# discord/lilliput

Measured on NVIDIA H100. Metric: images_per_sec_1080p_jpeg_to_256x256_jpeg_q85, higher is better.
Workload: dtype u8

## Files before the change

### lilliput_b200/csrc/jpeg_huff_parallel.cu

```cuda
#include <cstdlib>

#include "common.cuh"
#include "kernels.cuh"

namespace lp {

__device__ unsigned long long g_huff_phase[8];
#define LP_PHASE_MARK(k)                                             \
    do {                                                             \
        if (threadIdx.x == 0) {                                      \
            const long long now_ = clock64();                        \
            atomicAdd(&g_huff_phase[k], (unsigned long long)(now_ - s_tphase)); \
            s_tphase = now_;                                         \
        }                                                            \
    } while (0)

constexpr uint32_t kMinSubBits = 1024;
constexpr uint32_t kSubPerThread = 1;
#ifndef LP_HUFF_THREADS
#define LP_HUFF_THREADS 512
#endif
constexpr int kHuffThreads = LP_HUFF_THREADS;

__constant__ uint8_t c_zigzag_p[64] = {0,  1,  8,  16, 9,  2,  3,  10, 17, 24, 32, 25, 18, 11, 4,  5,
                                       12, 19, 26, 33, 40, 48, 41, 34, 27, 20, 13, 6,  7,  14, 21, 28,
                                       35, 42, 49, 56, 57, 50, 43, 36, 29, 22, 15, 23, 30, 37, 44, 51,
                                       58, 59, 52, 45, 38, 31, 39, 46, 53, 60, 61, 54, 47, 55, 62, 63};


template <int THREADS>
__device__ __forceinline__ uint32_t block_excl_scan(uint32_t v, uint32_t* total, uint32_t* warp_sums) {
    const int lane = threadIdx.x & 31, wid = threadIdx.x >> 5;
    uint32_t inc = v;
#pragma unroll
    for (int o = 1; o < 32; o <<= 1) {
        const uint32_t t = __shfl_up_sync(0xffffffffu, inc, o);
        if (lane >= o) inc += t;
    }
    if (lane == 31) warp_sums[wid] = inc;
    __syncthreads();
    if (wid == 0) {
        uint32_t s = lane < THREADS / 32 ? warp_sums[lane] : 0;
#pragma unroll
        for (int o = 1; o < 32; o <<= 1) {
            const uint32_t t = __shfl_up_sync(0xffffffffu, s, o);
            if (lane >= o) s += t;
        }
        if (lane < THREADS / 32) warp_sums[lane] = s;
    }
    __syncthreads();
    const uint32_t base = wid ? warp_sums[wid - 1] : 0;
    *total = warp_sums[THREADS / 32 - 1];
    __syncthreads();
    return base + inc - v;
}


__global__ void __launch_bounds__(kHuffThreads)
    jpeg_unstuff_kernel(JpegDecodeItem* items, const uint8_t* scan, uint8_t* clean) {
    __shared__ uint32_t warp_sums[kHuffThreads / 32];
    __shared__ uint32_t s_end;
    __shared__ __align__(16) uint8_t stage[kHuffThreads * 16 + 16];
    JpegDecodeItem& it = items[blockIdx.x];
    const uint8_t* src = scan + it.scan_off;
    const uint32_t len = it.scan_len;
    uint8_t* dst = clean + it.clean_off;
    const int tid = threadIdx.x, lane = tid & 31;
    if (it.restart_interval != 0 || it.nscans != 0) return;
    if (it.status != 0) {
        if (tid == 0) it.clean_len = 0;
        return;
    }
    if (tid == 0) s_end = len;
    __syncthreads();
    const uint32_t mis = (uint32_t)(reinterpret_cast<uintptr_t>(src) & 15);
    const uint8_t* abase = src - mis;
    uint32_t carry = 0;
    uint32_t end = len;
    constexpr uint32_t kTile = kHuffThreads * 16;
    for (uint32_t t0 = 0; t0 < mis + end; t0 += kTile) {
        const uint32_t aoff = t0 + (uint32_t)tid * 16;
        const int64_t i0 = (int64_t)aoff - (int64_t)mis;
        uint4 w = make_uint4(0, 0, 0, 0);
        if (aoff < mis + len + 16) w = *reinterpret_cast<const uint4*>(abase + aoff);
        uint32_t prev = __shfl_up_sync(0xffffffffu, w.w >> 24, 1);
        uint32_t next = __shfl_down_sync(0xffffffffu, w.x & 0xffu, 1);
        if (lane == 0) prev = i0 > 0 ? src[i0 - 1] : 0;
        if (lane == 31) next = (i0 + 16 < (int64_t)len) ? src[i0 + 16] : 0xD9u;
        const uint32_t ws[4] = {w.x, w.y, w.z, w.w};
        uint32_t m00[4], mff[4];
#pragma unroll
        for (int q = 0; q < 4; q++) {
            m00[q] = __vcmpeq4(ws[q], 0u);
            mff[q] = __vcmpeq4(ws[q], 0xFFFFFFFFu);
        }
        const uint32_t prev_ff = prev == 0xFFu ? 0xFFu : 0u, next_00 = next == 0x00u ? 0xFF000000u : 0u;
        uint32_t drop16 = 0, mark16 = 0;
#pragma unroll
        for (int q = 0; q < 4; q++) {
            const uint32_t pff = (mff[q] << 8) | (q ? mff[q - 1] >> 24 : prev_ff);
            const uint32_t n00 = (m00[q] >> 8) | (q < 3 ? m00[q + 1] << 24 : next_00);
            const uint32_t d = m00[q] & pff, mk = mff[q] & ~n00;
            drop16 |= (((d & 0x01010101u) * 0x01020408u) >> 24 & 0xFu) << (4 * q);
            mark16 |= (((mk & 0x01010101u) * 0x01020408u) >> 24 & 0xFu) << (4 * q);
        }
        const int64_t lo = -i0, hi = (int64_t)len - i0;
        uint32_t valid16 = 0xFFFFu;
        if (lo > 0) valid16 &= lo >= 16 ? 0u : (0xFFFFu << lo);
        if (hi < 16) valid16 &= hi <= 0 ? 0u : (0xFFFFu >> (16 - hi));
        if (lo >= 0 && lo < 16) drop16 &= ~(1u << (int)lo);
        if (hi >= 1 && hi <= 16) {
            const int kl = (int)hi - 1;
            if (((ws[kl >> 2] >> (8 * (kl & 3))) & 0xFFu) == 0xFFu) mark16 |= 1u << kl;
        }
        mark16 &= valid16;
        const uint32_t my_marker = mark16 ? (uint32_t)(i0 + (__ffs(mark16) - 1)) : 0xFFFFFFFFu;
        if (__syncthreads_or(my_marker != 0xFFFFFFFFu)) {
            if (my_marker != 0xFFFFFFFFu) atomicMin(&s_end, my_marker);
            __syncthreads();
            end = s_end;
        }
        uint32_t keep = valid16 & ~drop16;
        {
            const int64_t he = (int64_t)end - i0;
            if (he < 16) keep &= he <= 0 ? 0u : (0xFFFFu >> (16 - he));
        }
        uint8_t bsrc[16];
#pragma unroll
        for (int k = 0; k < 16; k++) bsrc[k] = (uint8_t)(ws[k >> 2] >> (8 * (k & 3)));
        const uint32_t cnt = __popc(keep);
        uint32_t total;
        const uint32_t ex = block_excl_scan<kHuffThreads>(cnt, &total, warp_sums);
        {
            uint32_t o = ex;
#pragma unroll
            for (int k = 0; k < 16; k++)
                if (keep & (1u << k)) stage[o++] = bsrc[k];
        }
        __syncthreads();
        uint8_t* d = dst + carry;
        const uint32_t head = min(total, (uint32_t)((4 - (reinterpret_cast<uintptr_t>(d) & 3)) & 3));
        const uint32_t nwords = (total - head) >> 2;
        const uint32_t tail0 = head + (nwords << 2);
        if ((uint32_t)tid < head) d[tid] = stage[tid];
        for (uint32_t j = tid; j < nwords; j += kHuffThreads) {
            const uint8_t* q = stage + head + 4 * j;
            *reinterpret_cast<uint32_t*>(d + head + 4 * j) = (uint32_t)q[0] | ((uint32_t)q[1] << 8) | ((uint32_t)q[2] << 16) | ((uint32_t)q[3] << 24);
        }
        if (tail0 + tid < total) d[tail0 + tid] = stage[tail0 + tid];
        carry += total;
        __syncthreads();
    }
    if (tid == 0) it.clean_len = carry;
    for (uint32_t k = tid; k < 32; k += kHuffThreads) dst[carry + k] = 0;
}


struct alignas(8) SubState {
    uint32_t p;
    uint32_t phase;
};

constexpr int kDcBits = 9, kAcBits = kHuffAcLookBits;

struct HuffShared {
    uint16_t dc_look[4][1 << kDcBits];
    uint16_t ac_look[4][1 << kAcBits];
    uint16_t ac_sub[4 * kHuffLongPrefixes][16];
    int32_t maxcode[8][18];
    int32_t valoffset[8][17];
    uint8_t vals[8][256];
    uint8_t zz[64];
    uint8_t blk_dc[16], blk_ac[16];
    uint8_t blk_comp[16], blk_bx[16], blk_by[16];
    uint32_t two_tables, n_first;
    uint32_t dcb_first, dcb_rest, acb_first, acb_rest;
};

struct BitWin {
    const uint32_t* w;
    uint32_t w0, w1;
    uint32_t nextw;
    uint32_t bo;
    __device__ __forceinline__ void init(const uint8_t* s, uint32_t p) {
        const uint32_t* base = reinterpret_cast<const uint32_t*>(s) + (p >> 5);
        w0 = __byte_perm(base[0], 0, 0x0123);
        w1 = __byte_perm(base[1], 0, 0x0123);
        nextw = base[2];
        w = base + 3;
        bo = p & 31;
    }
    __device__ __forceinline__ void refill() {
        if (bo >= 32) {
            w0 = w1;
            w1 = __byte_perm(nextw, 0, 0x0123);
            nextw = *w++;
            bo -= 32;
        }
    }
    __device__ __forceinline__ uint32_t peek() const { return __funnelshift_l(w1, w0, bo); }
    __device__ __forceinline__ void skip(int n) { bo += n; }
};

template <bool WRITE, bool TWO>
__device__ __forceinline__ void decode_span_t(const HuffShared& hs, const uint8_t* s, uint32_t& p, uint32_t limit,
                                            uint32_t end_bits, uint32_t& phase, uint32_t& nslots, int nb,
                                            uint64_t pos, uint64_t total_slots, const JpegDecodeItem* it,
                                            int16_t* coef, int16_t* dcdiff, int* status) {
    uint32_t blk = phase >> 6, z = phase & 63;
    const uint32_t z_start = z;
    uint32_t closed = 0;
    int32_t bits_left = (int32_t)(limit - p);
    const int32_t own_floor = (int32_t)limit - (int32_t)end_bits;
    bool own = z_start == 0;
    BitWin bw;
    bw.init(s, p);
    int16_t* dstblk = nullptr;
    bool inside = false;
    int16_t* dcp = nullptr;
    int mx = 0, my = 0;
    uint32_t blocks_left = 0;
    bool bad = false;
    int16_t* coef_base = nullptr;
    const uint32_t zzb = (uint32_t)__cvta_generic_to_shared(&hs.zz[0]);
    auto set_mcu = [&]() {
        const int rmx = mx - it->roi_mx0, rmy = my - it->roi_my0, rcx = it->roi_mcx;
        inside = (unsigned)rmx < (unsigned)rcx && (unsigned)rmy < (unsigned)it->roi_mcy;
        dstblk = coef_base + ((size_t)rmy * rcx + rmx) * ((size_t)nb * 64);
    };
    if (WRITE) {
        if (pos >= total_slots) {
            nslots = 0;
            return;
        }
        blocks_left = (uint32_t)((total_slots - pos + z_start) >> 6);
        coef_base = coef + it->coef_off;
        const uint32_t mcu = (uint32_t)((pos >> 6) / (uint32_t)nb);
        const uint32_t mcus_x = (uint32_t)it->mcus_x;
        mx = (int)(mcu % mcus_x);
        my = (int)(mcu / mcus_x);
        set_mcu();
        dstblk += blk * 64;
        dcp = dcdiff + (pos >> 6);
    }
    const uint32_t n_first = hs.n_first, dcbF = hs.dcb_first, dcbR = hs.dcb_rest, acbF = hs.acb_first, acbR = hs.acb_rest;
    uint32_t dcb, acb;
    auto set_tables = [&]() {
        if (TWO) {
            dcb = blk < n_first ? dcbF : dcbR;
            acb = blk < n_first ? acbF : acbR;
        } else {
            dcb = (uint32_t)__cvta_generic_to_shared(&hs.dc_look[hs.blk_dc[blk]][0]);
            acb = (uint32_t)__cvta_generic_to_shared(&hs.ac_look[hs.blk_ac[blk]][0]);
        }
    };
    set_tables();
    while (bits_left > 0 || (WRITE && own && z != 0 && bits_left > own_floor)) {
        bw.refill();
        const uint32_t top = bw.peek();
        const bool isdc = z == 0;
        const uint32_t idx = isdc ? (top >> (32 - kDcBits)) : (top >> (32 - kAcBits));
        int e;
        asm volatile("ld.shared.s16 %0, [%1];" : "=r"(e) : "r"((isdc ? dcb : acb) + idx * 2u));
        if (__builtin_expect(e <= 0, 0)) {
            if (e < 0) {
                e = hs.ac_sub[e & 0x7FFF][(top >> (32 - kAcBits - 4)) & 15u];
            } else {
                const int t = isdc ? hs.blk_dc[blk] : 4 + hs.blk_ac[blk];
                int len = (isdc ? kDcBits : kAcBits) + 1;
                int code = (int)(top >> (32 - len));
                while (len <= 16 && code > hs.maxcode[t][len]) {
                    len++;
                    code = (int)(top >> (32 - len));
                }
                if (len <= 16) e = (len << 8) | hs.vals[t][(code + hs.valoffset[t][len]) & 0xFF];
            }
            if (e == 0) {
                if (WRITE) {
                    *status = -3;
                    break;
                }
                bw.skip(1);
                bits_left -= 1;
                continue;
            }
        }
        const int len = e >> 8, sym = e & 0xFF;
        const uint32_t r = (uint32_t)sym >> 4, sz = (uint32_t)sym & 15;
        const bool ez = (sz == 0) && !isdc;
        const uint32_t adv = ez ? (r == 15 ? 16u : 64u) : r + 1;
        const uint32_t zt = z + adv;
        const int used = len + (ez ? 0 : (int)sz);
        if (WRITE) {
            const uint32_t t2 = top << len;
            const uint32_t raw = __funnelshift_l(t2, 0u, sz);
            const int val = (int)raw + ((int)t2 >= 0 ? (int)((0xFFFFFFFFu << sz) + 1u) : 0);
            uint32_t zi;
            asm volatile("ld.shared.u8 %0, [%1];" : "=r"(zi) : "r"(zzb + ((zt - 1u) & 63u)));
            int16_t* const where = isdc ? dcp : dstblk + zi;
            const bool inblk = zt <= 64;
            bad |= !ez && !inblk;
            if (isdc && inside) {
                uint4* const q = reinterpret_cast<uint4*>(dstblk);
#pragma unroll
                for (int k = 0; k < 8; k++) q[k] = make_uint4(0, 0, 0, 0);
            }
            if (!ez && inblk && own && (isdc || inside)) *where = (int16_t)val;
        }
        bw.skip(used);
        bits_left -= used;
        const bool fin = zt >= 64;
        z = fin ? 0u : zt;
        if (WRITE) own |= fin;
        if (!WRITE) {
            closed += fin ? 1u : 0u;
            const uint32_t nxt = blk + 1 == (uint32_t)nb ? 0u : blk + 1;
            blk = fin ? nxt : blk;
            set_tables();
        } else if (fin) {
            closed++;
            blk++;
            dstblk += 64;
            if (blk == (uint32_t)nb) {
                blk = 0;
                if (++mx == it->mcus_x) {
                    mx = 0;
                    my++;
                }
                set_mcu();
            }
            set_tables();
            if (--blocks_left == 0) break;
            dcp++;
        }
    }
    if (WRITE && bad) *status = -3;
    p = limit - (uint32_t)bits_left;
    phase = (blk << 6) | z;
    nslots = closed * 64 + z - z_start;
}

template <bool WRITE>
__device__ __forceinline__ void decode_span(const HuffShared& hs, const uint8_t* s, uint32_t& p, uint32_t limit,
                                            uint32_t end_bits, uint32_t& phase, uint32_t& nslots, int nb,
                                            uint64_t pos, uint64_t total_slots, const JpegDecodeItem* it,
                                            int16_t* coef, int16_t* dcdiff, int* status) {
    if (hs.two_tables)
        decode_span_t<WRITE, true>(hs, s, p, limit, end_bits, phase, nslots, nb, pos, total_slots, it, coef, dcdiff, status);
    else
        decode_span_t<WRITE, false>(hs, s, p, limit, end_bits, phase, nslots, nb, pos, total_slots, it, coef, dcdiff, status);
}

__device__ __forceinline__ void dc_prefix_pass(const JpegDecodeItem& it, int16_t* coef, const int16_t* dcdiff, int nb,
                                               uint32_t* warp_sums) {
    const int tid = threadIdx.x;
    constexpr int kDcRun = 8;
    const uint32_t mcus_x = (uint32_t)it.mcus_x;
    const int roi_mx0 = it.roi_mx0, roi_my0 = it.roi_my0, roi_mcx = it.roi_mcx, roi_mcy = it.roi_mcy;
    int koff = 0;
    for (int c = 0; c < it.ncomp; c++) {
        const uint32_t bpc = (uint32_t)(it.h[c] * it.v[c]);
        const uint32_t nblk = mcus_x * (uint32_t)it.mcus_y * bpc;
        const int16_t* dsrc = dcdiff + koff;
        int16_t* cdst = coef + it.coef_off + (size_t)koff * 64;
        uint32_t dc_before = 0;
        for (uint32_t base = 0; base < nblk; base += kHuffThreads * kDcRun) {
            const uint32_t j0 = base + (uint32_t)tid * kDcRun;
            const uint32_t mcu0 = j0 / bpc, kk0 = j0 % bpc;
            int d[kDcRun];
            uint32_t sum = 0;
            {
                uint32_t mcu = mcu0, kk = kk0;
#pragma unroll
                for (int r = 0; r < kDcRun; r++) {
                    d[r] = j0 + r < nblk ? dsrc[(size_t)mcu * nb + kk] : 0;
                    sum += (uint32_t)d[r];
                    if (++kk == bpc) {
                        kk = 0;
                        mcu++;
                    }
                }
            }
            uint32_t total;
            const uint32_t ex = block_excl_scan<kHuffThreads>(sum, &total, warp_sums);
            uint32_t run = dc_before + ex;
            dc_before += total;
            uint32_t mcu = mcu0, kk = kk0;
            int mx = (int)(mcu0 % mcus_x) - roi_mx0, my = (int)(mcu0 / mcus_x) - roi_my0;
#pragma unroll
            for (int r = 0; r < kDcRun; r++) {
                run += (uint32_t)d[r];
                if (j0 + r < nblk && (unsigned)mx < (unsigned)roi_mcx && (unsigned)my < (unsigned)roi_mcy)
                    cdst[(((size_t)my * roi_mcx + mx) * nb + kk) * 64] = (int16_t)(int)run;
                if (++kk == bpc) {
                    kk = 0;
                    mcu++;
                    if (++mx == (int)mcus_x - roi_mx0) {
                        mx = -roi_mx0;
                        my++;
                    }
                }
            }
        }
        koff += (int)bpc;
    }
}

#ifndef LP_HUFF_MIN_CTAS
#define LP_HUFF_MIN_CTAS 3
#endif
__global__ void __launch_bounds__(kHuffThreads, LP_HUFF_MIN_CTAS)
    jpeg_huff_sync_kernel(JpegDecodeItem* items, const JpegHuffSet* tables, const uint8_t* clean,
                          SubState* states_all, uint32_t* nslots_all, int16_t* coef, int16_t* dcdiff_all,
                          uint32_t sub_per_thread) {
    __shared__ HuffShared hs;
    __shared__ uint32_t warp_sums[kHuffThreads / 32];
    __shared__ uint32_t s_carry;
    __shared__ int s_status;
    JpegDecodeItem& it = items[blockIdx.x];
    const int tid = threadIdx.x;
    if (it.status != 0 || it.restart_interval != 0 || it.nscans != 0) return;
    __shared__ long long s_tphase;
    if (tid == 0) s_tphase = clock64();
    {
        const JpegHuffSet* g = tables + it.table_set;
        for (int i = tid; i < 8 * 18; i += kHuffThreads) (&hs.maxcode[0][0])[i] = (&g->maxcode[0][0])[i];
        for (int i = tid; i < 8 * 17; i += kHuffThreads) (&hs.valoffset[0][0])[i] = (&g->valoffset[0][0])[i];
        for (int i = tid; i < 8 * 256; i += kHuffThreads) (&hs.vals[0][0])[i] = (&g->vals[0][0])[i];
        for (int i = tid; i < 4 * (1 << kDcBits); i += kHuffThreads) (&hs.dc_look[0][0])[i] = (&g->look[0][0])[i];
        for (int i = tid; i < 4 * (1 << kAcBits); i += kHuffThreads) (&hs.ac_look[0][0])[i] = 0;
        if (tid < 64) hs.zz[tid] = c_zigzag_p[tid];
        if (tid == 0) {
            int k = 0;
            for (int c = 0; c < it.ncomp; c++)
                for (int j = 0; j < it.h[c] * it.v[c]; j++, k++) {
                    hs.blk_dc[k] = (uint8_t)it.td[c];
                    hs.blk_ac[k] = (uint8_t)it.ta[c];
                    hs.blk_comp[k] = (uint8_t)c;
                    hs.blk_bx[k] = (uint8_t)(j % it.h[c]);
                    hs.blk_by[k] = (uint8_t)(j / it.h[c]);
                }
            const int nfirst = it.h[0] * it.v[0];
            bool two = true;
            for (int b = 0; b < k; b++) {
                const int ref = b < nfirst ? 0 : nfirst;
                if (hs.blk_dc[b] != hs.blk_dc[ref] || hs.blk_ac[b] != hs.blk_ac[ref]) two = false;
            }
            const int rest = nfirst < k ? nfirst : 0;
            hs.two_tables = two;
            hs.n_first = (uint32_t)nfirst;
            hs.dcb_first = (uint32_t)__cvta_generic_to_shared(&hs.dc_look[hs.blk_dc[0]][0]);
            hs.acb_first = (uint32_t)__cvta_generic_to_shared(&hs.ac_look[hs.blk_ac[0]][0]);
            hs.dcb_rest = (uint32_t)__cvta_generic_to_shared(&hs.dc_look[hs.blk_dc[rest]][0]);
            hs.acb_rest = (uint32_t)__cvta_generic_to_shared(&hs.ac_look[hs.blk_ac[rest]][0]);
            s_status = 0;
            s_carry = 0;
        }
    }
    __syncthreads();
    {
        const JpegHuffSet* g = tables + it.table_set;
        for (int i = tid; i < 4 * (1 << kAcBits); i += kHuffThreads) {
            const int t = i >> kAcBits, idx = i & ((1 << kAcBits) - 1);
            uint16_t e = g->look[4 + t][idx >> (kAcBits - 9)];
            if (!e) {
                for (int len = 10; len <= kAcBits; len++) {
                    const int code = idx >> (kAcBits - len);
                    if (code <= hs.maxcode[4 + t][len]) {
                        e = (uint16_t)((len << 8) | hs.vals[4 + t][(code + hs.valoffset[4 + t][len]) & 0xFF]);
                        break;
                    }
                }
            }
            hs.ac_look[t][idx] = e;
        }
        for (int i = tid; i < 4 * kHuffLongPrefixes * 16; i += kHuffThreads)
            (&hs.ac_sub[0][0])[i] = (&g->long_sub[0][0][0])[i];
    }
    __syncthreads();
    if (tid < 4 * kHuffLongPrefixes) {
        const uint32_t pfx = (tables + it.table_set)->long_prefix[tid / kHuffLongPrefixes][tid % kHuffLongPrefixes];
        if (pfx < (1u << kAcBits)) hs.ac_look[tid / kHuffLongPrefixes][pfx] = (uint16_t)(0x8000u | (uint32_t)tid);
    }
    __syncthreads();
    int nb = 0;
    for (int c = 0; c < it.ncomp; c++) nb += it.h[c] * it.v[c];
    const uint8_t* s = clean + it.clean_off;
    const uint32_t total_bits = it.clean_len * 8u;
    uint32_t kSubBits = (total_bits + kHuffThreads * sub_per_thread - 1) / (kHuffThreads * sub_per_thread);
    kSubBits = max(kMinSubBits, (kSubBits + 31u) & ~31u);
    const uint32_t nsub = (total_bits + kSubBits - 1) / kSubBits;
    SubState* st = states_all + it.state_off;
    uint32_t* ns = nslots_all + it.state_off;
    uint32_t* list_a = reinterpret_cast<uint32_t*>(st + nsub);
    uint32_t* list_b = list_a + nsub;
    const uint64_t total_slots = (uint64_t)it.mcus_x * it.mcus_y * nb * 64;
    int16_t* dcdiff = dcdiff_all + it.dcdiff_off;

    LP_PHASE_MARK(0);
    for (uint32_t i = tid; i < nsub; i += kHuffThreads) {
        uint32_t p = i * kSubBits, phase = 0, n = 0;
        const uint32_t limit = min((i + 1) * kSubBits, total_bits);
        decode_span<false>(hs, s, p, limit, total_bits, phase, n, nb, 0, 0, nullptr, nullptr, nullptr, nullptr);
        st[i] = SubState{p, phase};
        ns[i] = n;
    }
    __syncthreads();
    LP_PHASE_MARK(1);
    uint32_t* cur_list = list_a;
    uint32_t* nxt_list = list_b;
    uint32_t cur_count = nsub > 0 ? nsub - 1 : 0;
    bool first_round = true;
    uint32_t rounds = 0;
    while (cur_count > 0) {
        rounds++;
        if (tid == 0) s_carry = 0;
        __syncthreads();
        for (uint32_t k = tid; k < cur_count; k += kHuffThreads) {
            const uint32_t i = first_round ? k + 1 : cur_list[k];
            const uint64_t in64 = *reinterpret_cast<volatile uint64_t*>(&st[i - 1]);
            const SubState in{(uint32_t)in64, (uint32_t)(in64 >> 32)};
            const SubState old = st[i];
            uint32_t p = in.p, phase = in.phase, n = 0;
            const uint32_t limit = min((i + 1) * kSubBits, total_bits);
            if (p < limit) decode_span<false>(hs, s, p, limit, total_bits, phase, n, nb, 0, 0, nullptr, nullptr, nullptr, nullptr);
            ns[i] = n;
            if (p != old.p || phase != old.phase) {
                *reinterpret_cast<volatile uint64_t*>(&st[i]) = ((uint64_t)phase << 32) | p;
                if (i + 1 < nsub) nxt_list[atomicAdd(&s_carry, 1u)] = i + 1;
            }
        }
        __syncthreads();
        cur_count = s_carry;
        __syncthreads();
        uint32_t* t = cur_list;
        cur_list = nxt_list;
        nxt_list = t;
        first_round = false;
    }
    if (tid == 0) it.pad_ = rounds;
    LP_PHASE_MARK(2);
    SubState* cur = st;
    uint64_t slots_before = 0;
    for (uint32_t base = 0; base < nsub; base += kHuffThreads) {
        const uint32_t i = base + tid;
        const uint32_t v = i < nsub ? ns[i] : 0;
        uint32_t total;
        const uint32_t ex = block_excl_scan<kHuffThreads>(v, &total, warp_sums);
        const uint64_t pos = slots_before + ex;
        slots_before += total;
        if (i < nsub) {
            uint32_t p = i == 0 ? 0u : cur[i - 1].p;
            uint32_t phase = i == 0 ? 0u : cur[i - 1].phase;
            uint32_t n = 0;
            const uint32_t limit = min((i + 1) * kSubBits, total_bits);
            int status = 0;
            if (pos < total_slots &&
                (uint32_t)(pos % ((uint64_t)nb * 64)) != ((phase >> 6) * 64 + (phase & 63)))
                status = -3;
            if (!status && p < limit)
                decode_span<true>(hs, s, p, limit, total_bits, phase, n, nb, pos, total_slots, &it, coef, dcdiff, &status);
            if (status) s_status = status;
        }
    }
    if (tid == 0 && slots_before < total_slots) s_status = -3;
    __syncthreads();
    if (s_status) {
        if (tid == 0) it.status = s_status;
        return;
    }
    LP_PHASE_MARK(3);
    dc_prefix_pass(it, coef, dcdiff, nb, warp_sums);
    LP_PHASE_MARK(4);
    if (tid == 0) atomicAdd(&g_huff_phase[5], 1ull);
}



int jpeg_huff_phase_clocks(unsigned long long out[8], int reset) {
    LP_CUDA_OK(cudaDeviceSynchronize());
    LP_CUDA_OK(cudaMemcpyFromSymbol(out, g_huff_phase, sizeof(unsigned long long) * 8));
    if (reset) {
        unsigned long long z[8] = {0, 0, 0, 0, 0, 0, 0, 0};
        LP_CUDA_OK(cudaMemcpyToSymbol(g_huff_phase, z, sizeof(z)));
    }
    return LP_OK;
}

int jpeg_huff_parallel_slots() {
    int dev = 0, sms = 0, per_sm = 0;
    if (cudaGetDevice(&dev) != cudaSuccess) return 0;
    cudaDeviceGetAttribute(&sms, cudaDevAttrMultiProcessorCount, dev);
    cudaOccupancyMaxActiveBlocksPerMultiprocessor(&per_sm, jpeg_huff_sync_kernel, kHuffThreads, 0);
    return sms * per_sm;
}

int jpeg_huff_parallel_launch(const JpegHuffParallelArgs& a, cudaStream_t st) {
    if (a.n <= 0) return LP_OK;
    static const uint32_t spt = getenv("LP_HUFF_SPT") ? (uint32_t)atoi(getenv("LP_HUFF_SPT")) : kSubPerThread;
    jpeg_unstuff_kernel<<<a.n, kHuffThreads, 0, st>>>(a.items, a.scan, a.clean);
    g_launches++;
    LP_CUDA_OK(cudaGetLastError());
    jpeg_huff_sync_kernel<<<a.n, kHuffThreads, 0, st>>>(a.items, a.tables, a.clean,
                                                       reinterpret_cast<SubState*>(a.states), a.nslots, a.coef,
                                                       a.dcdiff, spt);
    g_launches++;
    LP_CUDA_OK(cudaGetLastError());
    return LP_OK;
}

}
```

### lilliput_b200/csrc/jpeg_types.h

```cpp
#pragma once
#include <stdint.h>

namespace lp {

struct JpegScanDesc {
    uint32_t data_off, data_len;
    int32_t ns;
    int32_t ci[3], td[3], ta[3];
    int32_t Ss, Se, Ah, Al;
    int32_t restart_interval;
    int32_t table_set;
    int32_t progressive;
};

struct JpegDecodeItem {
    uint64_t scan_off;
    uint32_t scan_len;
    uint32_t table_set;
    uint64_t coef_off;
    uint64_t frame_off;
    int32_t width, height, ncomp;
    int32_t mcus_x, mcus_y, restart_interval;
    int32_t h[3], v[3];
    int32_t bw[3], bh[3];
    int32_t dw[3], dh[3];
    uint32_t block_off[3];
    int32_t tile_mcx, tile_mcy, tiles_x;
    uint16_t qt[3][64];
    int32_t td[3], ta[3];
    int32_t status;
    int32_t frame_channels;
    uint64_t clean_off;
    uint64_t state_off;
    uint64_t dcdiff_off;
    uint32_t clean_len;
    uint32_t pad_;
    int32_t roi_mx0, roi_my0, roi_mcx, roi_mcy;
    int32_t win_x0, win_y0, win_w, win_h;
    uint32_t win_stride;
    uint32_t nscans;
};

constexpr int kHuffAcLookBits = 12;
constexpr int kHuffLongPrefixes = 16;
struct JpegHuffSet {
    uint16_t look[8][512];
    int32_t maxcode[8][18];
    int32_t valoffset[8][17];
    uint8_t vals[8][256];
    uint16_t long_prefix[4][kHuffLongPrefixes];
    uint16_t long_sub[4][kHuffLongPrefixes][16];
};

}
```

Baseline: 50750.

## Decode AC symbol pairs in the Huffman sync pass via packed 32-bit lookup

The AC lookup table grows from 16-bit to 32-bit entries. The upper half stores a precomputed two-symbol step (combined bit length and zigzag advance), so the non-writing synchronization pass can skip over two AC symbols per iteration. The direct AC lookup width drops from 12 to 11 bits to keep shared memory in check, and the long-code prefix and sub-table sizes are adjusted to match. This adds an extra table-building pass per block and longer-code fallbacks at a smaller table width, and it relies on the host filling the reshaped long_sub and long_prefix layouts with the new constants.

```diff
diff --git a/lilliput_b200/csrc/jpeg_huff_look.h b/lilliput_b200/csrc/jpeg_huff_look.h
--- /dev/null
+++ b/lilliput_b200/csrc/jpeg_huff_look.h
@@ -0,0 +1,46 @@
+#pragma once
+#include <stdint.h>
+
+#include "jpeg_types.h"
+
+#ifdef __CUDACC__
+#define LP_HL_FN __host__ __device__ inline
+#else
+#define LP_HL_FN inline
+#endif
+
+namespace lp {
+
+LP_HL_FN uint32_t huff_ac_advance(uint32_t sym) {
+    const uint32_t r = sym >> 4;
+    return (sym & 15) ? r + 1 : (r == 15 ? 16u : 64u);
+}
+
+LP_HL_FN uint32_t huff_ac_single(const JpegHuffSet& g, int t, uint32_t idx) {
+    uint32_t e = g.look[4 + t][idx >> (kHuffAcLookBits - 9)];
+    if (!e) {
+        for (int len = 10; len <= kHuffAcLookBits; len++) {
+            const int code = (int)(idx >> (kHuffAcLookBits - len));
+            if (code <= g.maxcode[4 + t][len]) {
+                e = ((uint32_t)len << 8) | g.vals[4 + t][(code + g.valoffset[4 + t][len]) & 0xFF];
+                break;
+            }
+        }
+    }
+    return e;
+}
+
+LP_HL_FN uint32_t huff_ac_pair(const uint16_t* look16, uint32_t idx) {
+    const uint32_t e1 = look16[2 * idx];
+    if (e1 == 0 || (e1 & 0x8000u)) return 0;
+    const uint32_t sym1 = e1 & 0xFF, used1 = (e1 >> 8) + (sym1 & 15);
+    const uint32_t adv1 = huff_ac_advance(sym1);
+    if (adv1 >= 64 || used1 >= (uint32_t)kHuffAcLookBits) return 0;
+    const uint32_t e2 = look16[2 * ((idx << used1) & ((1u << kHuffAcLookBits) - 1))];
+    if (e2 == 0 || (e2 & 0x8000u)) return 0;
+    const uint32_t sym2 = e2 & 0xFF, len2 = e2 >> 8;
+    if (used1 + len2 > (uint32_t)kHuffAcLookBits) return 0;
+    return ((used1 + len2 + (sym2 & 15)) << 11) | ((adv1 + huff_ac_advance(sym2)) << 4) | (sym2 & 15);
+}
+
+}
diff --git a/lilliput_b200/csrc/jpeg_huff_parallel.cu b/lilliput_b200/csrc/jpeg_huff_parallel.cu
--- a/lilliput_b200/csrc/jpeg_huff_parallel.cu
+++ b/lilliput_b200/csrc/jpeg_huff_parallel.cu
@@ -1,6 +1,7 @@
 #include <cstdlib>
 
 #include "common.cuh"
+#include "jpeg_huff_look.h"
 #include "kernels.cuh"
 
 namespace lp {
@@ -165,8 +166,8 @@
 
 struct HuffShared {
     uint16_t dc_look[4][1 << kDcBits];
-    uint16_t ac_look[4][1 << kAcBits];
-    uint16_t ac_sub[4 * kHuffLongPrefixes][16];
+    uint32_t ac_look[4][1 << kAcBits];
+    uint16_t ac_sub[4 * kHuffLongPrefixes][1 << kHuffLongSubBits];
     int32_t maxcode[8][18];
     int32_t valoffset[8][17];
     uint8_t vals[8][256];
@@ -259,12 +260,21 @@
         bw.refill();
         const uint32_t top = bw.peek();
         const bool isdc = z == 0;
-        const uint32_t idx = isdc ? (top >> (32 - kDcBits)) : (top >> (32 - kAcBits));
         int e;
-        asm volatile("ld.shared.s16 %0, [%1];" : "=r"(e) : "r"((isdc ? dcb : acb) + idx * 2u));
+        uint32_t ea = 0;
+        if (WRITE) {
+            asm volatile("ld.shared.s16 %0, [%1];"
+                         : "=r"(e)
+                         : "r"(isdc ? dcb + (top >> (32 - kDcBits)) * 2u : acb + (top >> (32 - kAcBits)) * 4u));
+        } else {
+            int ed;
+            asm volatile("ld.shared.s16 %0, [%1];" : "=r"(ed) : "r"(dcb + (top >> (32 - kDcBits)) * 2u));
+            asm volatile("ld.shared.u32 %0, [%1];" : "=r"(ea) : "r"(acb + (top >> (32 - kAcBits)) * 4u));
+            e = isdc ? ed : (int)(int16_t)ea;
+        }
         if (__builtin_expect(e <= 0, 0)) {
             if (e < 0) {
-                e = hs.ac_sub[e & 0x7FFF][(top >> (32 - kAcBits - 4)) & 15u];
+                e = hs.ac_sub[e & 0x7FFF][(top >> (32 - kAcBits - kHuffLongSubBits)) & ((1u << kHuffLongSubBits) - 1)];
             } else {
                 const int t = isdc ? hs.blk_dc[blk] : 4 + hs.blk_ac[blk];
                 int len = (isdc ? kDcBits : kAcBits) + 1;
@@ -289,8 +299,12 @@
         const uint32_t r = (uint32_t)sym >> 4, sz = (uint32_t)sym & 15;
         const bool ez = (sz == 0) && !isdc;
         const uint32_t adv = ez ? (r == 15 ? 16u : 64u) : r + 1;
-        const uint32_t zt = z + adv;
-        const int used = len + (ez ? 0 : (int)sz);
+        const uint32_t z1 = z + adv;
+        const int used1 = len + (ez ? 0 : (int)sz);
+        const uint32_t pr = isdc ? 0u : ea >> 16;
+        const bool take = !WRITE && pr != 0 && z1 < 64 && bits_left > used1;
+        const uint32_t zt = take ? z + ((pr >> 4) & 0x7Fu) : z1;
+        const int used = take ? (int)(pr >> 11) : used1;
         if (WRITE) {
             const uint32_t t2 = top << len;
             const uint32_t raw = __funnelshift_l(t2, 0u, sz);
@@ -428,7 +442,6 @@
         for (int i = tid; i < 8 * 17; i += kHuffThreads) (&hs.valoffset[0][0])[i] = (&g->valoffset[0][0])[i];
         for (int i = tid; i < 8 * 256; i += kHuffThreads) (&hs.vals[0][0])[i] = (&g->vals[0][0])[i];
         for (int i = tid; i < 4 * (1 << kDcBits); i += kHuffThreads) (&hs.dc_look[0][0])[i] = (&g->look[0][0])[i];
-        for (int i = tid; i < 4 * (1 << kAcBits); i += kHuffThreads) (&hs.ac_look[0][0])[i] = 0;
         if (tid < 64) hs.zz[tid] = c_zigzag_p[tid];
         if (tid == 0) {
             int k = 0;
@@ -460,27 +473,23 @@
     __syncthreads();
     {
         const JpegHuffSet* g = tables + it.table_set;
-        for (int i = tid; i < 4 * (1 << kAcBits); i += kHuffThreads) {
-            const int t = i >> kAcBits, idx = i & ((1 << kAcBits) - 1);
-            uint16_t e = g->look[4 + t][idx >> (kAcBits - 9)];
-            if (!e) {
-                for (int len = 10; len <= kAcBits; len++) {
-                    const int code = idx >> (kAcBits - len);
-                    if (code <= hs.maxcode[4 + t][len]) {
-                        e = (uint16_t)((len << 8) | hs.vals[4 + t][(code + hs.valoffset[4 + t][len]) & 0xFF]);
-                        break;
-                    }
-                }
-            }
-            hs.ac_look[t][idx] = e;
-        }
-        for (int i = tid; i < 4 * kHuffLongPrefixes * 16; i += kHuffThreads)
+        for (int i = tid; i < 4 * (1 << kAcBits); i += kHuffThreads)
+            hs.ac_look[i >> kAcBits][i & ((1 << kAcBits) - 1)] = huff_ac_single(*g, i >> kAcBits, i & ((1 << kAcBits) - 1));
+        for (int i = tid; i < 4 * kHuffLongPrefixes * (1 << kHuffLongSubBits); i += kHuffThreads)
             (&hs.ac_sub[0][0])[i] = (&g->long_sub[0][0][0])[i];
     }
     __syncthreads();
     if (tid < 4 * kHuffLongPrefixes) {
         const uint32_t pfx = (tables + it.table_set)->long_prefix[tid / kHuffLongPrefixes][tid % kHuffLongPrefixes];
-        if (pfx < (1u << kAcBits)) hs.ac_look[tid / kHuffLongPrefixes][pfx] = (uint16_t)(0x8000u | (uint32_t)tid);
+        if (pfx < (1u << kAcBits)) hs.ac_look[tid / kHuffLongPrefixes][pfx] = 0x8000u | (uint32_t)tid;
+    }
+    __syncthreads();
+    {
+        uint16_t* const look16 = reinterpret_cast<uint16_t*>(&hs.ac_look[0][0]);
+        for (int i = tid; i < 4 * (1 << kAcBits); i += kHuffThreads) {
+            uint16_t* const tab = look16 + 2 * ((i >> kAcBits) << kAcBits);
+            tab[2 * (i & ((1 << kAcBits) - 1)) + 1] = (uint16_t)huff_ac_pair(tab, i & ((1 << kAcBits) - 1));
+        }
     }
     __syncthreads();
     int nb = 0;
diff --git a/lilliput_b200/csrc/jpeg_types.h b/lilliput_b200/csrc/jpeg_types.h
--- a/lilliput_b200/csrc/jpeg_types.h
+++ b/lilliput_b200/csrc/jpeg_types.h
@@ -41,15 +41,16 @@
     uint32_t nscans;
 };
 
-constexpr int kHuffAcLookBits = 12;
-constexpr int kHuffLongPrefixes = 16;
+constexpr int kHuffAcLookBits = 11;
+constexpr int kHuffLongPrefixes = 8;
+constexpr int kHuffLongSubBits = 16 - kHuffAcLookBits;
 struct JpegHuffSet {
     uint16_t look[8][512];
     int32_t maxcode[8][18];
     int32_t valoffset[8][17];
     uint8_t vals[8][256];
     uint16_t long_prefix[4][kHuffLongPrefixes];
-    uint16_t long_sub[4][kHuffLongPrefixes][16];
+    uint16_t long_sub[4][kHuffLongPrefixes][1 << kHuffLongSubBits];
 };
 
 }
```

Result: no change. 50940, median of 6 (+0.4%).
